# fraunhoferhhi/vvenc

Measured on AMD Instinct MI355X. Metric: frames/sec + bit-exact vs CPU, 1080p/4K 10-bit preset=faster at 1/2/4/8 GPU, higher is better.
Workload: dtype i16; 1 GPU; BASELINE configs[1]: hot-path work lists RECORDED from the reference encoder (1920x1080 10-bit synthetic clip, 65 frames, preset faster; one picture per temporal layer), replayed resident in HBM: a step = one picture's integer-ME SAD windows + sub-pel SATD stages + table calls + fused TU transform/quant lists + DMVR lists on 5 HIP streams; steps follow the GOP's 1:1:2:4:8:16 layer mix from the key; hip_streams=5, sample_pairs_per_frame=175309451, coefficients_per_frame=6951461, recorded_calls_outside_the_lists=0

## Files before the change

### vvenc_amd/csrc/dmvr.hip

```cpp
#include "common.h"

namespace {

constexpr int DP = 24;

typedef uint32_t u32x4 __attribute__( ( ext_vector_type( 4 ) ) );
typedef short dmvrS2 __attribute__( ( ext_vector_type( 2 ) ) );
__device__ __forceinline__ int dmvrDot2( uint32_t a, uint32_t b, int c ) { return __builtin_amdgcn_sdot2( __builtin_bit_cast( dmvrS2, a ), __builtin_bit_cast( dmvrS2, b ), c, false ); }
__device__ __forceinline__ uint32_t dmvrPack( int lo, int hi ) { return ( ( uint32_t ) lo & 0xffffu ) | ( ( uint32_t ) hi << 16 ); }

__device__ __forceinline__ int divMaxQ7( long long N, long long D )
{
  int sign = 0, q = 0;
  if( N < 0 ) { sign = 1; N = -N; }
  D <<= 3;
  if( N >= D ) { N -= D; q++; }
  q <<= 1;
  D >>= 1;
  if( N >= D ) { N -= D; q++; }
  q <<= 1;
  if( N >= ( D >> 1 ) ) q++;
  return sign ? -q : q;
}

VVHIP_GROUP_REDUCE( dmvrGroupMin32, ( o < v ? o : v ) )

template<int dx, int dy>
__global__ void __launch_bounds__( 256 )
dmvrRefineKernel( const int16_t* __restrict__ ref0, int stride0, const int16_t* __restrict__ ref1, int stride1, const vvhip_dmvr_item* __restrict__ items, int n,
                  int bitDepth, vvhip_dmvr_result* __restrict__ out )
{
  __shared__ __attribute__( ( aligned( 16 ) ) ) int16_t sT[4][2][22 * DP];
  __shared__ __attribute__( ( aligned( 16 ) ) ) int16_t sR[4][2][20 * DP];
  __shared__ uint32_t sCost[4][32];
  struct __attribute__( ( packed, aligned( 2 ) ) ) U16 { u32x4 v; };
  struct __attribute__( ( packed, aligned( 2 ) ) ) U4 { uint32_t v; };
  const int wv = threadIdx.x >> 6, lane = threadIdx.x & 63;
  const int q = ( int ) gridDim.x >> 3, g = ( int ) blockIdx.x < ( q << 3 ) ? ( ( int ) blockIdx.x & 7 ) * q + ( ( int ) blockIdx.x >> 3 ) : ( int ) blockIdx.x;
  const int blk = g * 4 + wv;
  if( blk >= n ) return;
  const vvhip_dmvr_item it = items[blk];
  constexpr int bw = dx + 4, bh = dy + 4, segs = ( bw + 7 ) >> 3;
  const int sh1 = 4 - ( 10 - bitDepth ), of1 = 1 << ( sh1 - 1 );
  const int16_t* s0 = ref0 + it.ref0_off - 2 * stride0 - 2;
  const int16_t* s1 = ref1 + it.ref1_off - 2 * stride1 - 2;
// ... 19 lines not shown
      u32x4 o = A[q];
      if( fxs[q] )
      {
        const uint32_t w = dmvrPack( 16 - fxs[q], fxs[q] );
        const uint32_t e[5] = { A[q].x, A[q].y, A[q].z, A[q].w, B[q] };
        uint32_t r[4];
#pragma unroll
        for( int i = 0; i < 4; i++ )
          r[i] = dmvrPack( dmvrDot2( e[i], w, of1 ) >> sh1, dmvrDot2( __builtin_amdgcn_alignbit( e[i + 1], e[i], 16 ), w, of1 ) >> sh1 );
        o.x = r[0]; o.y = r[1]; o.z = r[2]; o.w = r[3];
      }
      *reinterpret_cast<u32x4*>( &sT[wv][0][at[q]] ) = o;
    }
  }
  DMVR_SYNC();
  {
    const int perList = bh * segs, jobs = 2 * perList;
    for( int jb = lane; jb < jobs; jb += 64 )
    {
      const int list = jb >= perList, rem = jb - list * perList, y = segs == 3 ? rem / 3 : rem >> 1, x0 = ( rem - y * segs ) * 8;
      const int fx = ( list ? it.frac1_x : it.frac0_x ) & 15, fy = ( list ? it.frac1_y : it.frac0_y ) & 15;
      const u32x4 a = *reinterpret_cast<const u32x4*>( &sT[wv][list][y * DP + x0] );
      u32x4 o = a;
      if( fy )
      {
        const u32x4 b = *reinterpret_cast<const u32x4*>( &sT[wv][list][( y + 1 ) * DP + x0] );
        const int rnd = fx ? 8 : of1, sh = fx ? 4 : sh1;
        const uint32_t w = dmvrPack( 16 - fy, fy );
        const uint32_t aw[4] = { a.x, a.y, a.z, a.w }, bw_[4] = { b.x, b.y, b.z, b.w };
        uint32_t r[4];
#pragma unroll
        for( int i = 0; i < 4; i++ )
          r[i] = dmvrPack( dmvrDot2( __builtin_amdgcn_perm( bw_[i], aw[i], 0x05040100u ), w, rnd ) >> sh, dmvrDot2( __builtin_amdgcn_perm( bw_[i], aw[i], 0x07060302u ), w, rnd ) >> sh );
        o.x = r[0]; o.y = r[1]; o.z = r[2]; o.w = r[3];
      }
      else if( !fx )
      {
        const int s = 10 - bitDepth;
        const uint32_t aw[4] = { a.x, a.y, a.z, a.w };
        uint32_t r[4];
#pragma unroll
        for( int i = 0; i < 4; i++ ) r[i] = dmvrPack( ( int ) ( int16_t ) ( aw[i] & 0xffffu ) << s, ( ( int ) aw[i] >> 16 ) << s );
        o.x = r[0]; o.y = r[1]; o.z = r[2]; o.w = r[3];
      }
      o.x ^= 0x80008000u; o.y ^= 0x80008000u; o.z ^= 0x80008000u; o.w ^= 0x80008000u;
      *reinterpret_cast<u32x4*>( &sR[wv][list][y * DP + x0] ) = o;
    }
  }
  DMVR_SYNC();
  {
    constexpr int rows = dy >> 1, dw = dx >> 1, PPW = 64 / rows;
    const int r = lane & ( rows - 1 ), slot = lane / rows;
#pragma unroll
    for( int pass = 0; pass < ( 15 + PPW - 1 ) / PPW; pass++ )
    {
      const int idx = pass * PPW + slot;
      const bool valid = idx < 15;
      const int iv = valid ? idx : 7, v3 = ( iv * 11 ) >> 5, ver = v3 - 2, hor = 2 * ( iv - 3 * v3 ) - 2;
      const uint32_t* p0 = reinterpret_cast<const uint32_t*>( &sR[wv][0][( 2 + 2 * r + ver ) * DP + 2 + hor] );
      const uint32_t* p1 = reinterpret_cast<const uint32_t*>( &sR[wv][1][( 2 + 2 * r - ver ) * DP + 2 - hor] );
      uint32_t sum = 0;
// ... 67 lines not shown
  }
#undef DMVR_SYNC
}

}

extern "C" {

int vvhip_dmvr_refine_batch( vvhip_ctx* ctx, const int16_t* d_ref0, int stride0, const int16_t* d_ref1, int stride1, const vvhip_dmvr_item* d_items, int n,
                             int dx, int dy, int bit_depth, vvhip_dmvr_result* d_out )
{
  if( !ctx ) return VVHIP_E_ARG;
  if( n < 0 || ( dx != 8 && dx != 16 ) || ( dy != 8 && dy != 16 ) || bit_depth < 8 || bit_depth > 10 || ( n && ( !d_ref0 || !d_ref1 || !d_items || !d_out ) ) )
    return vvhip_fail( ctx, VVHIP_E_ARG, "vvhip_dmvr_refine_batch: sub-block %dx%d (8 or 16 per side, DMVR_SUBCU_SIZE 16) bitDepth %d (<= 10: the bilinear taps keep 10-bit precision)", dx, dy, bit_depth );
  if( n == 0 ) return VVHIP_OK;
  const dim3 grid( ( n + 3 ) / 4 ), block( 256 );
  if( dx == 16 && dy == 16 )     hipLaunchKernelGGL( ( dmvrRefineKernel<16, 16> ), grid, block, 0, ctx->stream, d_ref0, stride0, d_ref1, stride1, d_items, n, bit_depth, d_out );
  else if( dx == 16 )            hipLaunchKernelGGL( ( dmvrRefineKernel<16, 8> ), grid, block, 0, ctx->stream, d_ref0, stride0, d_ref1, stride1, d_items, n, bit_depth, d_out );
  else if( dy == 16 )            hipLaunchKernelGGL( ( dmvrRefineKernel<8, 16> ), grid, block, 0, ctx->stream, d_ref0, stride0, d_ref1, stride1, d_items, n, bit_depth, d_out );
  else                           hipLaunchKernelGGL( ( dmvrRefineKernel<8, 8> ), grid, block, 0, ctx->stream, d_ref0, stride0, d_ref1, stride1, d_items, n, bit_depth, d_out );
  VVHIP_LAUNCH_CHECK( ctx );
  return VVHIP_OK;
}

}
```

### vvenc_amd/csrc/me.hip

```cpp
#include <stdlib.h>
#ifndef VVHIP_ME_HU
#define VVHIP_ME_HU 2
#endif
#ifndef VVHIP_ME_STAGE_WAVES
#define VVHIP_ME_STAGE_WAVES 6
#endif
#ifndef VVHIP_ME_ITEM_WAVES
#define VVHIP_ME_ITEM_WAVES 8
#endif
#include <string.h>
#include <algorithm>
#include <vector>
#include "common.h"

struct vvhip_me_plan
{
  int bitDepth = 0, nCands = 0, nStages = 0, nItems = 0, nMaskItems = 0, maxPlane = 0;
  int wavesInt = 0, wavesStage = 0, wavesItem = 0, wavesItemMain = 0, ldsInt = 0, ldsStage = 0;
  int intBig = 0, ldsIntSmall = 0;
  int intLarge = 0, ldsIntMid = 0;
  bool stageAtomic = false;
  bool intSplit = false;
  bool timing = false; hipEvent_t ev[5] = { nullptr, nullptr, nullptr, nullptr, nullptr };
  int stageSetWaves[6] = { 0, 0, 0, 0, 0, 0 }, stageSetLds[6] = { 0, 0, 0, 0, 0, 0 };
  void* d_blob = nullptr;
  const void* d_intJobs = nullptr; const void* d_cands = nullptr; const void* d_candOut = nullptr; const void* d_stageJobs = nullptr; const void* d_stageOrder = nullptr; const void* d_stageWaves = nullptr;
  const void* d_items = nullptr; const void* d_itemOrder = nullptr; const void* d_itemWaves = nullptr; const void* d_tapTables = nullptr; const void* d_maskItems = nullptr;
};

namespace {

typedef uint32_t u32x2 __attribute__( ( ext_vector_type( 2 ) ) );
// ... 688 lines not shown
      for( int q = 0; q < CW / 2; q++ ) { bits |= va[q] | vb[q]; const uint32_t df = pkSub( va[q], vb[q] ); acc = ( uint32_t ) dot2( df, df, ( int ) acc ); }
    }
  }
  if( __builtin_amdgcn_ballot_w64( ( bits & 0xf000f000u ) != 0 ) == 0ull ) return acc;
  uint64_t sse = 0;
  for( int it = nIt; it > 0; it--, pa += stepA, pb += stepB )
  {
    uint32_t va[CW / 2], vb[CW / 2];
    itemChunk<CW>( pa, pb, va, vb );
#pragma unroll
    for( int q = 0; q < CW / 2; q++ ) { const int d0 = lo16( va[q] ) - lo16( vb[q] ), d1 = hi16( va[q] ) - hi16( vb[q] ); sse += ( uint64_t ) ( ( int64_t ) d0 * d0 ) + ( uint64_t ) ( ( int64_t ) d1 * d1 ); }
  }
  return sse;
}

template<bool GEN>
__device__ __forceinline__ void itemBody( const MePlanes& P, const MeArgs& a, int wave, int nItems )
{
  __shared__ const int16_t* planeL[16];
  __shared__ int strideL[16];
  const WaveSpan span = a.itemWaves[wave];
  const int lane = threadIdx.x & 63;
  if( lane < 16 ) { planeL[lane] = P.p[lane]; strideL[lane] = P.stride[lane]; }
  __builtin_amdgcn_fence( __ATOMIC_ACQ_REL, "wavefront" ); __builtin_amdgcn_wave_barrier();
  if( GEN && span.count < 0 ) { maskItemBody( a, span, nItems, planeL, strideL, lane ); return; }
  const vvhip_me_item first = a.items[span.first];
  const int w = first.width, h = first.height, func = first.func, ss = func == VVHIP_DF_SAD ? first.sub_shift : 0;
  if( func == VVHIP_DF_SAD || func == VVHIP_DF_SSE )
  {
    const int cw = w >= 8 ? 8 : ( ( !GEN || w >= 4 ) ? 4 : 2 ), lprShift = ( 31 - __builtin_clz( w ) ) - ( 31 - __builtin_clz( cw ) ), lpr = 1 << lprShift, rowsEff = h >> ss, chunks = rowsEff * lpr;
    const int lpcShift = chunks >= 64 ? 6 : 31 - __builtin_clz( chunks ), lpc = 1 << lpcShift;
    const int teams = 64 >> lpcShift, lt = lane & ( lpc - 1 ), team = lane >> lpcShift;
    for( int i0 = 0; i0 < span.count; i0 += teams )
    {
      const int ii = i0 + team;
      const bool valid = ii < span.count;
      const int idx = a.itemOrder[span.first + ( valid ? ii : 0 )];
      const vvhip_me_item it = a.items[span.first + ( valid ? ii : 0 )];
      const int16_t* po = planeL[it.org_plane] + it.org_off; const int os = strideL[it.org_plane] ? strideL[it.org_plane] : w;
      const int16_t* pc = planeL[it.cur_plane] + it.cur_off; const int cs = strideL[it.cur_plane] ? strideL[it.cur_plane] : w;
      const int r0 = lt >> lprShift, s0 = lt & ( lpr - 1 ), rowStep = lpc >> lprShift;
      const int16_t* pa = po + ( ptrdiff_t ) ( r0 << ss ) * os + s0 * cw;
      const int16_t* pb = pc + ( ptrdiff_t ) ( r0 << ss ) * cs + s0 * cw;
      const ptrdiff_t stepA = ( ptrdiff_t ) ( rowStep << ss ) * os, stepB = ( ptrdiff_t ) ( rowStep << ss ) * cs;
      const int nIt = chunks >> lpcShift;
      const bool isSad = func == VVHIP_DF_SAD;
      const uint64_t mine = cw == 8 ? itemSadSse<8>( isSad, pa, pb, stepA, stepB, nIt ) : ( ( !GEN || cw == 4 ) ? itemSadSse<4>( isSad, pa, pb, stepA, stepB, nIt ) : itemSadSse<2>( isSad, pa, pb, stepA, stepB, nIt ) );
      if( isSad ) { const uint32_t t = vvhipGroupSum32( ( uint32_t ) mine, lpc, lane ); if( valid && lt == 0 ) a.itemCost[idx] = ( uint64_t ) t << ss; }
      else        { const uint64_t t = vvhipGroupSum64( mine, lpc, lane ); if( valid && lt == 0 ) a.itemCost[idx] = t; }
    }
    return;
  }
  const int kind = GEN ? hadTileKind( w, h, func == VVHIP_DF_HAD_FAST ) : ( w == 4 ? TK_4x4 : ( ( func == VVHIP_DF_HAD_FAST && ( w & 31 ) == 0 ) ? TK_16F : TK_8x8 ) );
  if( !GEN && kind == TK_4x4 )
  {
    const int ii = lane;
    const bool valid = ii < span.count;
    const int idx = a.itemOrder[span.first + ( valid ? ii : 0 )];
    const vvhip_me_item it = a.items[span.first + ( valid ? ii : 0 )];
    const int16_t* qa = planeL[it.org_plane] + it.org_off; const int os = strideL[it.org_plane] ? strideL[it.org_plane] : w;
    const int16_t* qb = planeL[it.cur_plane] + it.cur_off; const int cs = strideL[it.cur_plane] ? strideL[it.cur_plane] : w;
    int d[16]; uint32_t sad = 0;
#pragma unroll
    for( int r = 0; r < 4; r++ )
    {
      const u32x2 x = ld8( qa + ( ptrdiff_t ) r * os ), z = ld8( qb + ( ptrdiff_t ) r * cs );
      d[4 * r] = lo16( x.x ) - lo16( z.x ); d[4 * r + 1] = hi16( x.x ) - hi16( z.x ); d[4 * r + 2] = lo16( x.y ) - lo16( z.y ); d[4 * r + 3] = hi16( x.y ) - hi16( z.y );
      if( func == VVHIP_DF_HAD_2SAD ) { sad = __builtin_amdgcn_sad_u16( x.x ^ BIAS, z.x ^ BIAS, sad ); sad = __builtin_amdgcn_sad_u16( x.y ^ BIAS, z.y ^ BIAS, sad ); }
    }
    const uint64_t tot = hadamard4x4( d ), s2 = 2ull * sad;
    if( valid ) a.itemCost[idx] = ( func == VVHIP_DF_HAD_2SAD && s2 < tot ) ? s2 : tot;
    return;
  }
  __shared__ uint32_t accAll[4][128];
  uint32_t* accL = accAll[( threadIdx.x >> 6 ) & 3];
  accL[lane] = 0; accL[64 + lane] = 0;
  __builtin_amdgcn_fence( __ATOMIC_ACQ_REL, "wavefront" ); __builtin_amdgcn_wave_barrier();
  const int PW = GEN ? tileW( kind ) : ( kind == TK_16F ? 16 : 8 ), PH = GEN ? tileH( kind ) : PW, LT = GEN ? tileLanes( kind ) : 8, log2LT = GEN ? 31 - __builtin_clz( LT ) : 3;
  const int log2TX = ( 31 - __builtin_clz( w ) ) - ( 31 - __builtin_clz( PW ) ), tilesX = 1 << log2TX, log2Slots = log2TX + ( 31 - __builtin_clz( h ) ) - ( 31 - __builtin_clz( PH ) ) + log2LT;
  const int slotsPerItem = 1 << log2Slots, total = span.count * slotsPerItem;
  for( int s0 = 0; s0 < total; s0 += 64 )
  {
    const int sl = s0 + lane;
    const bool valid = sl < total;
    const int sv = valid ? sl : 0, ii = sv >> log2Slots, rem = sv & ( slotsPerItem - 1 ), t = rem >> log2LT, r = rem & ( LT - 1 );
    const vvhip_me_item it = a.items[span.first + ii];
// ... 28 lines not shown
      }
      else
      {
        uint32_t xw[4], zw[4];
        if( GEN && kind == TK_4x8 )
        {
          const u32x2 xa = ld8( qa + ( ptrdiff_t ) ( 2 * r ) * os ), xb = ld8( qa + ( ptrdiff_t ) ( 2 * r + 1 ) * os ), za = ld8( qb + ( ptrdiff_t ) ( 2 * r ) * cs ), zb = ld8( qb + ( ptrdiff_t ) ( 2 * r + 1 ) * cs );
          xw[0] = xa.x; xw[1] = xa.y; xw[2] = xb.x; xw[3] = xb.y; zw[0] = za.x; zw[1] = za.y; zw[2] = zb.x; zw[3] = zb.y;
        }
        else
        {
          const int row = ( GEN && kind == TK_16x8 ) ? ( r & 7 ) : r, col = ( GEN && kind == TK_16x8 ) ? 8 * ( r >> 3 ) : 0;
          const u32x4 x = ld16( qa + ( ptrdiff_t ) row * os + col ), z = ld16( qb + ( ptrdiff_t ) row * cs + col );
          xw[0] = x.x; xw[1] = x.y; xw[2] = x.z; xw[3] = x.w; zw[0] = z.x; zw[1] = z.y; zw[2] = z.z; zw[3] = z.w;
        }
        if( func == VVHIP_DF_HAD_2SAD )
        {
#pragma unroll
          for( int i = 0; i < 4; i++ ) sad = __builtin_amdgcn_sad_u16( xw[i] ^ BIAS, zw[i] ^ BIAS, sad );
        }
        sres = hadTeamPk( xw, zw, r, GEN ? LT : 8, GEN ? kind : TK_8x8, lane );
      }
      if( func == VVHIP_DF_HAD_2SAD ) sad = vvhipGroupSum32( sad, GEN ? LT : 8, lane );
    }
    if( valid && r == 0 ) { atomicAdd( &accL[ii], sres ); if( func == VVHIP_DF_HAD_2SAD ) atomicAdd( &accL[64 + ii], sad ); }
  }
  __builtin_amdgcn_fence( __ATOMIC_ACQ_REL, "wavefront" ); __builtin_amdgcn_wave_barrier();
  if( lane < span.count )
  {
    const int idx = a.itemOrder[span.first + lane];
    const uint64_t tot = accL[lane], s2 = 2ull * accL[64 + lane];
    a.itemCost[idx] = ( func == VVHIP_DF_HAD_2SAD && s2 < tot ) ? s2 : tot;
  }
}

template<int K0, int K1, bool GEN>
__global__ void __launch_bounds__( 128 ) __attribute__( ( amdgpu_waves_per_eu( VVHIP_ME_STAGE_WAVES, VVHIP_ME_STAGE_WAVES ) ) )
meStageKernel( MePlanes P, MeArgs a, int firstWave, int nWaves, int ldsPerWave )
{
  extern __shared__ __attribute__( ( aligned( 16 ) ) ) int16_t meLds[];
  __shared__ uint32_t pairCost[16];
  const int wv = __builtin_amdgcn_readfirstlane( ( int ) ( threadIdx.x >> 6 ) ), wave = blockIdx.x * 2 + wv;
  if( wave < nWaves ) stageBody<K0, K1, GEN>( P, a, a.stageWaves[firstWave + wave], meLds + wv * ( ldsPerWave >> 1 ), pairCost, wv );
}

__global__ void __launch_bounds__( 256 )
meIntKernel( MePlanes P, MeArgs a, int nBig, int ldsSmall, int blockBase )
// ... 57 lines not shown
  return mePlanCreate( ctx, L, bit_depth, max_window, out );
}

int vvhip_me_plan_create_lists( vvhip_ctx* ctx, const vvhip_me_lists* lists, int bit_depth, int max_window, vvhip_me_plan** out )
{
  if( !ctx || !lists ) return VVHIP_E_ARG;
  return mePlanCreate( ctx, *lists, bit_depth, max_window, out );
}

static int mePlanCreate( vvhip_ctx* ctx, const vvhip_me_lists& L, int bit_depth, int max_window, vvhip_me_plan** out )
{
  if( !ctx || !out ) return VVHIP_E_ARG;
  *out = nullptr;
  const vvhip_me_int_job* int_jobs = L.int_jobs; const vvhip_me_cand* cands = L.cands; const vvhip_me_stage_job* stage_jobs = L.stage_jobs; const vvhip_me_item* items = L.items;
  const vvhip_me_mask_item* mask_items = L.mask_items;
  const int n_int_jobs = L.n_int_jobs, n_cands = L.n_cands, n_stage_jobs = L.n_stage_jobs, n_items = L.n_items, n_mask = L.n_mask_items;
  if( n_int_jobs < 0 || n_cands < 0 || n_stage_jobs < 0 || n_items < 0 || n_mask < 0 || ( n_int_jobs && ( !int_jobs || !cands ) ) || ( n_stage_jobs && !stage_jobs ) || ( n_items && !items ) || ( n_mask && !mask_items ) )
    return vvhip_fail( ctx, VVHIP_E_ARG, "vvhip_me_plan_create: bad lists" );
  if( n_cands >= ( 1 << 24 ) ) return vvhip_fail( ctx, VVHIP_E_ARG, "vvhip_me_plan_create: %d candidates (the schedule packs the output-list position into 24 bits)", n_cands );
  if( n_stage_jobs > ST_STAGE_MASK ) return vvhip_fail( ctx, VVHIP_E_ARG, "vvhip_me_plan_create: %d stage jobs (the schedule packs the stage index into 22 bits)", n_stage_jobs );
  if( bit_depth < 8 || bit_depth > 10 ) return vvhip_fail( ctx, VVHIP_E_UNSUPPORTED, "vvhip_me_plan_create: bit depth %d (the packed Hadamard tile covers <= 10)", bit_depth );
  if( max_window <= 0 ) max_window = 24;
  auto shapeOk = []( int w, int h, int minW, int minH ) { return isPow2( w ) && isPow2( h ) && w >= minW && h >= minH && w <= 128 && h <= 128; };

  std::vector<IntJob> ij; std::vector<PlanCand> pc; std::vector<int32_t> candOut;
  int ldsInt = 0;
  static const bool dedupe = !( getenv( "VVHIP_ME_DEDUPE" ) && atoi( getenv( "VVHIP_ME_DEDUPE" ) ) == 0 );
  static const int candCap = getenv( "VVHIP_ME_CAND_CAP" ) ? atoi( getenv( "VVHIP_ME_CAND_CAP" ) ) : 16;
  for( int i = 0; i < n_int_jobs; i++ )
  {
    const vvhip_me_int_job& s = int_jobs[i];
// ... 175 lines not shown
      }
    }
  }
  for( int k = 0, first = 0; k < 6; first += setWaves[k], k++ )
    for( int w = 0; w < setWaves[k]; w++ )
    {
      const WaveSpan& sp = stWaves[first + w];
      const int u = stOrder[sp.first];
      const vvhip_me_stage_job& s = stage_jobs[u & ST_STAGE_MASK];
      if( dealOf( s ) != 0 ) continue;
      const int sib = ( w & 1 ) ? w - 1 : w + 1;
      if( sp.count != unitsOf( s ) / 2 || sib >= setWaves[k] || stWaves[first + sib].count != sp.count || ( stOrder[stWaves[first + sib].first] & ( ST_STAGE_MASK | ( 3 << ST_VAR_SHIFT ) ) ) != ( u & ( ST_STAGE_MASK | ( 3 << ST_VAR_SHIFT ) ) ) )
        return vvhip_fail( ctx, VVHIP_E_HIP, "vvhip_me_plan_create: schedule error (the units of stage %d are not one workgroup)", u & ST_STAGE_MASK );
    }

  std::vector<int32_t> itOrder( ( size_t ) n_items + n_mask ); std::vector<WaveSpan> itWaves;
  for( int i = 0; i < n_items; i++ )
  {
    const vvhip_me_item& s = items[i];
    const bool fOk = s.func == VVHIP_DF_SAD || s.func == VVHIP_DF_SSE || s.func == VVHIP_DF_HAD || s.func == VVHIP_DF_HAD_FAST || s.func == VVHIP_DF_HAD_2SAD;
    if( !shapeOk( s.width, s.height, 2, 2 ) || !fOk || s.org_plane > 15 || s.cur_plane > 15 || s.sub_shift > 1 || ( s.sub_shift && ( s.func != VVHIP_DF_SAD || s.height < 2 ) ) )
      return vvhip_fail( ctx, VVHIP_E_ARG, "vvhip_me_plan_create: item %d (func %d, %dx%d)", i, s.func, s.width, s.height );
    itOrder[i] = i;
  }
  auto itemGen = [&]( int i ) { const auto& s = items[i]; if( s.func == VVHIP_DF_SAD || s.func == VVHIP_DF_SSE ) return s.width < 4;
                                const int kind = hadTileKind( s.width, s.height, s.func == VVHIP_DF_HAD_FAST ); return !( kind == TK_8x8 || kind == TK_16F || ( kind == TK_4x4 && s.width == 4 && s.height == 4 ) ); };
  auto itemKey = [&]( int i ) { const auto& s = items[i]; return ( itemGen( i ) ? 0l : 1l << 48 ) | ( ( long ) s.width << 32 ) | ( ( long ) s.height << 16 ) | ( s.func << 8 ) | s.sub_shift; };
  std::stable_sort( itOrder.begin(), itOrder.begin() + n_items, [&]( int a, int b ) { return itemKey( a ) > itemKey( b ); } );
  int wavesItemMain = 0;
  for( int i = 0; i < n_items; )
  {
    const vvhip_me_item& s0 = items[itOrder[i]];
    int lanesPer;
    if( s0.func == VVHIP_DF_SAD || s0.func == VVHIP_DF_SSE ) { const int cw = s0.width >= 8 ? 8 : ( s0.width >= 4 ? 4 : 2 ); lanesPer = ( s0.height >> ( s0.func == VVHIP_DF_SAD ? s0.sub_shift : 0 ) ) * ( s0.width / cw ); }
    else { const int kind = hadTileKind( s0.width, s0.height, s0.func == VVHIP_DF_HAD_FAST ); lanesPer = kind == TK_4x4 ? 1 : ( s0.width / tileW( kind ) ) * ( s0.height / tileH( kind ) ) * tileLanes( kind ); }
    if( lanesPer > 64 ) lanesPer = 64;
    const int perWave = std::max( 1, 64 / lanesPer );
    int count = 0;
    while( i + count < n_items && count < perWave && itemKey( itOrder[i + count] ) == itemKey( itOrder[i] ) ) count++;
// ... 80 lines not shown
    for( int k = 0; k < 9; k++ )
    {
      if( !( ( u.j.mask >> k ) & 1 ) ) continue;
      tx[k] = ( rxT[k] + u.j.base_qx ) * u.j.i_frac * 4; ty[k] = ( ( u.j.i_frac == 2 ? ryH[k] : ryQ[k] ) + u.j.base_qy ) * u.j.i_frac * 4;
      int v = 0; while( v < nHor && u.hx[v] != tx[k] ) v++;
      if( v == nHor ) u.hx[nHor++] = ( int16_t ) tx[k];
      var[k] = v; cnt[v]++; nPos++;
    }
    u.nHor = ( uint8_t ) nHor; u.nPos = ( uint8_t ) nPos; u.cnt0 = ( uint8_t ) cnt[0]; u.cnt1 = ( uint8_t ) cnt[1]; u.cnt2 = ( uint8_t ) cnt[2];
    int slot[3] = { 0, cnt[0], cnt[0] + cnt[1] };
    for( int k = 0; k < 9; k++ ) if( ( u.j.mask >> k ) & 1 ) u.pos[slot[var[k]]++] = k | ( ( tx[k] + 64 ) << 8 ) | ( ( ty[k] + 64 ) << 20 );
  }
  std::vector<vvhip_me_item> itSorted( n_items );
  for( int i = 0; i < n_items; i++ ) itSorted[i] = items[itOrder[i]];
  std::vector<vvhip_me_mask_item> mkSorted( n_mask );
  for( int i = 0; i < n_mask; i++ ) { mkSorted[i] = mask_items[itOrder[n_items + i]]; itOrder[n_items + i] += n_items; }
  const std::vector<int32_t> tapTab = stageTapTables( bit_depth );
  auto pad = []( size_t b ) { return ( b + 255 ) & ~( size_t ) 255; };
  const size_t bInt = pad( ij.size() * sizeof( IntJob ) ), bCand = pad( pc.size() * sizeof( PlanCand ) ), bCandO = pad( candOut.size() * 4 ), bSt = pad( stUnits.size() * sizeof( StageUnit ) ),
               bStO = pad( stOrder.size() * 4 ), bStW = pad( stWaves.size() * sizeof( WaveSpan ) ), bIt = pad( ( size_t ) n_items * sizeof( vvhip_me_item ) ), bItO = pad( itOrder.size() * 4 ),
               bItW = pad( itWaves.size() * sizeof( WaveSpan ) ), bMk = pad( mkSorted.size() * sizeof( vvhip_me_mask_item ) );
  const size_t bTap = pad( tapTab.size() * 4 );
  const size_t total = bInt + bCand + bCandO + bSt + bStO + bStW + bIt + bItO + bItW + bTap + bMk + 256;
  std::vector<char> host( total, 0 );
  size_t o = 0;
  auto put = [&]( const void* src, size_t bytes, size_t padded ) { const size_t at = o; if( bytes ) memcpy( host.data() + o, src, bytes ); o += padded; return at; };
  const size_t oInt = put( ij.data(), ij.size() * sizeof( IntJob ), bInt ), oCand = put( pc.data(), pc.size() * sizeof( PlanCand ), bCand ), oCandO = put( candOut.data(), candOut.size() * 4, bCandO ),
               oSt = put( stUnits.data(), stUnits.size() * sizeof( StageUnit ), bSt ), oStO = put( stOrder.data(), stOrder.size() * 4, bStO ),
               oStW = put( stWaves.data(), stWaves.size() * sizeof( WaveSpan ), bStW ), oIt = put( itSorted.data(), ( size_t ) n_items * sizeof( vvhip_me_item ), bIt ),
               oItO = put( itOrder.data(), itOrder.size() * 4, bItO ), oItW = put( itWaves.data(), itWaves.size() * sizeof( WaveSpan ), bItW ), oTap = put( tapTab.data(), tapTab.size() * 4, bTap ),
               oMk = put( mkSorted.data(), mkSorted.size() * sizeof( vvhip_me_mask_item ), bMk );
  vvhip_me_plan* p = new vvhip_me_plan;
  hipError_t e = hipMalloc( &p->d_blob, total );
  if( e != hipSuccess ) { delete p; return vvhip_fail( ctx, VVHIP_E_NOMEM, "vvhip_me_plan_create: hipMalloc( %zu ): %s", total, hipGetErrorString( e ) ); }
  e = hipMemcpyAsync( p->d_blob, host.data(), total, hipMemcpyHostToDevice, ctx->stream );
  if( e == hipSuccess ) e = hipStreamSynchronize( ctx->stream );
  if( e != hipSuccess ) { ( void ) hipFree( p->d_blob ); delete p; return vvhip_fail( ctx, VVHIP_E_HIP, "vvhip_me_plan_create: upload: %s", hipGetErrorString( e ) ); }
  char* b = static_cast<char*>( p->d_blob );
  p->d_intJobs = b + oInt; p->d_cands = b + oCand; p->d_candOut = b + oCandO; p->d_stageJobs = b + oSt; p->d_stageOrder = b + oStO; p->d_stageWaves = b + oStW; p->d_items = b + oIt; p->d_itemOrder = b + oItO; p->d_itemWaves = b + oItW; p->d_tapTables = b + oTap; p->d_maskItems = b + oMk;
  p->bitDepth = bit_depth; p->nCands = n_cands; p->nStages = n_stage_jobs; p->nItems = n_items; p->nMaskItems = n_mask; p->maxPlane = maxPlane; p->stageAtomic = hasAtomic;
  p->wavesInt = ( int ) ij.size(); p->wavesStage = ( int ) stWaves.size(); p->wavesItem = ( int ) itWaves.size(); p->wavesItemMain = wavesItemMain;
  p->ldsInt = ( ldsInt + 15 ) & ~15; p->ldsStage = ( ldsStage + 15 ) & ~15;
  for( int k = 0; k < 6; k++ ) { p->stageSetWaves[k] = setWaves[k]; p->stageSetLds[k] = setLds[k]; }
  p->intBig = intBig; p->ldsIntSmall = ( ldsIntSmall + 15 ) & ~15; p->intLarge = intLarge; p->ldsIntMid = ( ldsIntMid + 15 ) & ~15;
  p->intSplit = intBig > 0 && intBig < ( int ) ij.size() && p->ldsInt > 2 * 4 * p->ldsIntSmall && p->ldsInt > 32 * 1024;
  if( p->ldsInt > 160 * 1024 || p->ldsStage > 64 * 1024 )
  { ( void ) hipFree( p->d_blob ); delete p; return vvhip_fail( ctx, VVHIP_E_UNSUPPORTED, "vvhip_me_plan_create: %d / %d bytes of LDS per wave (max_window too large?)", ldsInt, ldsStage ); }
  *out = p;
  return VVHIP_OK;
}

void vvhip_me_plan_destroy( vvhip_ctx* ctx, vvhip_me_plan* plan )
{
  if( !plan ) return;
  if( ctx ) ( void ) hipStreamSynchronize( ctx->stream );
// ... 89 lines not shown
      }
      else hipLaunchKernelGGL( meIntKernel, dim3( ( unsigned ) plan->intBig ), dim3( 256 ), ( size_t ) plan->ldsInt, ctx->stream, P, a, plan->intBig, plan->ldsIntSmall, 0 );
      if( splitSmall && nSmall ) hipLaunchKernelGGL( meIntKernel, dim3( ( unsigned ) ( ( nSmall + 3 ) / 4 ) ), dim3( 256 ), ( size_t ) 4 * plan->ldsIntSmall, ctx->stream, P, a, plan->intBig, plan->ldsIntSmall, plan->intBig );
    }
  }
  if( tm ) VVHIP_CHECK_HIP( ctx, hipEventRecord( plan->ev[2], ctx->stream ) );
  if( tm ) VVHIP_CHECK_HIP( ctx, hipEventRecord( plan->ev[3], ctx->stream ) );
  if( plan->wavesItem && doItem )
  {
    const int nMain = plan->wavesItemMain, nGen = plan->wavesItem - nMain;
    static const int longSpans = getenv( "VVHIP_ME_ITEM_SPANS" ) ? atoi( getenv( "VVHIP_ME_ITEM_SPANS" ) ) : 1;
    auto launch = [&]( bool gen, int first, int n )
    {
      if( n <= 65536 )
      {
        if( gen ) hipLaunchKernelGGL( ( meItemKernel<4, true> ), dim3( ( unsigned ) ( ( n + 3 ) / 4 ) ), dim3( 256 ), 0, ctx->stream, P, a, plan->nItems, first, n, 1 );
        else      hipLaunchKernelGGL( ( meItemKernel<4, false> ), dim3( ( unsigned ) ( ( n + 3 ) / 4 ) ), dim3( 256 ), 0, ctx->stream, P, a, plan->nItems, first, n, 1 );
      }
      else
      {
        const int spw = longSpans < 1 ? 1 : longSpans, nw = ( n + spw - 1 ) / spw;
        if( gen ) hipLaunchKernelGGL( ( meItemKernel<1, true> ), dim3( ( unsigned ) nw ), dim3( 64 ), 0, ctx->stream, P, a, plan->nItems, first, n, spw );
        else      hipLaunchKernelGGL( ( meItemKernel<1, false> ), dim3( ( unsigned ) nw ), dim3( 64 ), 0, ctx->stream, P, a, plan->nItems, first, n, spw );
      }
    };
    if( nMain ) launch( false, 0, nMain );
    if( nGen ) launch( true, nMain, nGen );
  }
  VVHIP_LAUNCH_CHECK( ctx );
  if( tm ) VVHIP_CHECK_HIP( ctx, hipEventRecord( plan->ev[4], ctx->stream ) );
  return VVHIP_OK;
}

}
#endif
```

Measured before the change: 15530 frames/s.

## Early-exit DMVR on centre cost and deduplicate identical ME item calls

In DMVR, each wave first builds only the rows needed for the zero-offset SAD. If that centre cost is under the dx*dy threshold, it writes a zero refinement and returns, which skips interpolating the rest of the window and evaluating the other 14 search positions. In ME plan creation, items with the same operands are grouped so duplicate calls are computed once and the result is scattered to every output slot. A HAD item and a SAD item over the same block are also merged so one pass produces both costs. This adds host-side sorting at plan build time and indirect output lists on device, and it changes how item order is encoded, so correctness depends on the new index packing.

```diff
diff --git a/vvenc_amd/csrc/dmvr.hip b/vvenc_amd/csrc/dmvr.hip
--- a/vvenc_amd/csrc/dmvr.hip
+++ b/vvenc_amd/csrc/dmvr.hip
@@ -28,7 +28,7 @@
 template<int dx, int dy>
 __global__ void __launch_bounds__( 256 )
 dmvrRefineKernel( const int16_t* __restrict__ ref0, int stride0, const int16_t* __restrict__ ref1, int stride1, const vvhip_dmvr_item* __restrict__ items, int n,
-                  int bitDepth, vvhip_dmvr_result* __restrict__ out )
+                  int bitDepth, int centreFirst, vvhip_dmvr_result* __restrict__ out )
 {
   __shared__ __attribute__( ( aligned( 16 ) ) ) int16_t sT[4][2][22 * DP];
   __shared__ __attribute__( ( aligned( 16 ) ) ) int16_t sR[4][2][20 * DP];
@@ -78,37 +78,78 @@
     }
   }
   DMVR_SYNC();
+  const auto second = [&]( int list, int y, int x0 )
+  {
+    const int fx = ( list ? it.frac1_x : it.frac0_x ) & 15, fy = ( list ? it.frac1_y : it.frac0_y ) & 15;
+    const u32x4 a = *reinterpret_cast<const u32x4*>( &sT[wv][list][y * DP + x0] );
+    u32x4 o = a;
+    if( fy )
+    {
+      const u32x4 b = *reinterpret_cast<const u32x4*>( &sT[wv][list][( y + 1 ) * DP + x0] );
+      const int rnd = fx ? 8 : of1, sh = fx ? 4 : sh1;
+      const uint32_t w = dmvrPack( 16 - fy, fy );
+      const uint32_t aw[4] = { a.x, a.y, a.z, a.w }, bw_[4] = { b.x, b.y, b.z, b.w };
+      uint32_t r[4];
+#pragma unroll
+      for( int i = 0; i < 4; i++ )
+        r[i] = dmvrPack( dmvrDot2( __builtin_amdgcn_perm( bw_[i], aw[i], 0x05040100u ), w, rnd ) >> sh, dmvrDot2( __builtin_amdgcn_perm( bw_[i], aw[i], 0x07060302u ), w, rnd ) >> sh );
+      o.x = r[0]; o.y = r[1]; o.z = r[2]; o.w = r[3];
+    }
+    else if( !fx )
+    {
+      const int s = 10 - bitDepth;
+      const uint32_t aw[4] = { a.x, a.y, a.z, a.w };
+      uint32_t r[4];
+#pragma unroll
+      for( int i = 0; i < 4; i++ ) r[i] = dmvrPack( ( int ) ( int16_t ) ( aw[i] & 0xffffu ) << s, ( ( int ) aw[i] >> 16 ) << s );
+      o.x = r[0]; o.y = r[1]; o.z = r[2]; o.w = r[3];
+    }
+    o.x ^= 0x80008000u; o.y ^= 0x80008000u; o.z ^= 0x80008000u; o.w ^= 0x80008000u;
+    *reinterpret_cast<u32x4*>( &sR[wv][list][y * DP + x0] ) = o;
+  };
+  if( centreFirst )
+  {
+    constexpr int rows = dy >> 1, dw = dx >> 1, perList = rows * segs, restList = ( bh - rows ) * segs, ahead = 64 - 2 * perList;
+    const auto rest = [&]( int jb, int& list, int& y, int& x0 )
+    {
+      list = jb >= restList;
+      const int rem = jb - list * restList, k = segs == 3 ? rem / 3 : rem >> 1;
+      y = k < 2 ? k : k <= rows + 1 ? 2 * k - 1 : k + rows; x0 = ( rem - k * segs ) * 8;
+    };
+    {
+      int list, y, x0;
+      rest( lane - 2 * perList, list, y, x0 );
+      if( lane < 2 * perList ) { list = lane >= perList; const int rem = lane - list * perList, r = segs == 3 ? rem / 3 : rem >> 1; y = 2 + 2 * r; x0 = ( rem - r * segs ) * 8; }
+      if( lane < 2 * perList + 2 * restList ) second( list, y, x0 );
+    }
+    DMVR_SYNC();
+    uint32_t sum = 0;
+    if( lane < rows )
+    {
+      const uint32_t* p0 = reinterpret_cast<const uint32_t*>( &sR[wv][0][( 2 + 2 * lane ) * DP + 2] );
+      const uint32_t* p1 = reinterpret_cast<const uint32_t*>( &sR[wv][1][( 2 + 2 * lane ) * DP + 2] );
+#pragma unroll
+      for( int i = 0; i < dw; i++ ) sum = __builtin_amdgcn_sad_u16( p0[i], p1[i], sum );
+    }
+    const uint32_t s = ( uint32_t ) __builtin_amdgcn_readfirstlane( ( int ) vvhipGroupSum32( sum, rows, lane ) ), centre = s - ( s >> 2 );
+    if( centre < ( uint32_t ) ( dx * dy ) )
+    {
+      if( lane == 0 )
+      {
+        vvhip_dmvr_result r; r.mvd_x = 0; r.mvd_y = 0; r.pad = 0; r.min_cost = centre;
+        out[blk] = r;
+      }
+      return;
+    }
+    for( int jb = lane + ahead; jb < 2 * restList; jb += 64 ) { int list, y, x0; rest( jb, list, y, x0 ); second( list, y, x0 ); }
+  }
+  else
   {
     const int perList = bh * segs, jobs = 2 * perList;
     for( int jb = lane; jb < jobs; jb += 64 )
     {
-      const int list = jb >= perList, rem = jb - list * perList, y = segs == 3 ? rem / 3 : rem >> 1, x0 = ( rem - y * segs ) * 8;
-      const int fx = ( list ? it.frac1_x : it.frac0_x ) & 15, fy = ( list ? it.frac1_y : it.frac0_y ) & 15;
-      const u32x4 a = *reinterpret_cast<const u32x4*>( &sT[wv][list][y * DP + x0] );
-      u32x4 o = a;
-      if( fy )
-      {
-        const u32x4 b = *reinterpret_cast<const u32x4*>( &sT[wv][list][( y + 1 ) * DP + x0] );
-        const int rnd = fx ? 8 : of1, sh = fx ? 4 : sh1;
-        const uint32_t w = dmvrPack( 16 - fy, fy );
-        const uint32_t aw[4] = { a.x, a.y, a.z, a.w }, bw_[4] = { b.x, b.y, b.z, b.w };
-        uint32_t r[4];
-#pragma unroll
-        for( int i = 0; i < 4; i++ )
-          r[i] = dmvrPack( dmvrDot2( __builtin_amdgcn_perm( bw_[i], aw[i], 0x05040100u ), w, rnd ) >> sh, dmvrDot2( __builtin_amdgcn_perm( bw_[i], aw[i], 0x07060302u ), w, rnd ) >> sh );
-        o.x = r[0]; o.y = r[1]; o.z = r[2]; o.w = r[3];
-      }
-      else if( !fx )
-      {
-        const int s = 10 - bitDepth;
-        const uint32_t aw[4] = { a.x, a.y, a.z, a.w };
-        uint32_t r[4];
-#pragma unroll
-        for( int i = 0; i < 4; i++ ) r[i] = dmvrPack( ( int ) ( int16_t ) ( aw[i] & 0xffffu ) << s, ( ( int ) aw[i] >> 16 ) << s );
-        o.x = r[0]; o.y = r[1]; o.z = r[2]; o.w = r[3];
-      }
-      o.x ^= 0x80008000u; o.y ^= 0x80008000u; o.z ^= 0x80008000u; o.w ^= 0x80008000u;
-      *reinterpret_cast<u32x4*>( &sR[wv][list][y * DP + x0] ) = o;
+      const int list = jb >= perList, rem = jb - list * perList, y = segs == 3 ? rem / 3 : rem >> 1;
+      second( list, y, ( rem - y * segs ) * 8 );
     }
   }
   DMVR_SYNC();
@@ -206,11 +247,12 @@
   if( n < 0 || ( dx != 8 && dx != 16 ) || ( dy != 8 && dy != 16 ) || bit_depth < 8 || bit_depth > 10 || ( n && ( !d_ref0 || !d_ref1 || !d_items || !d_out ) ) )
     return vvhip_fail( ctx, VVHIP_E_ARG, "vvhip_dmvr_refine_batch: sub-block %dx%d (8 or 16 per side, DMVR_SUBCU_SIZE 16) bitDepth %d (<= 10: the bilinear taps keep 10-bit precision)", dx, dy, bit_depth );
   if( n == 0 ) return VVHIP_OK;
+  static const int centreFirst = []{ const char* e = getenv( "VVHIP_DMVR_CENTRE_FIRST" ); return e ? atoi( e ) != 0 : 1; }();
   const dim3 grid( ( n + 3 ) / 4 ), block( 256 );
-  if( dx == 16 && dy == 16 )     hipLaunchKernelGGL( ( dmvrRefineKernel<16, 16> ), grid, block, 0, ctx->stream, d_ref0, stride0, d_ref1, stride1, d_items, n, bit_depth, d_out );
-  else if( dx == 16 )            hipLaunchKernelGGL( ( dmvrRefineKernel<16, 8> ), grid, block, 0, ctx->stream, d_ref0, stride0, d_ref1, stride1, d_items, n, bit_depth, d_out );
-  else if( dy == 16 )            hipLaunchKernelGGL( ( dmvrRefineKernel<8, 16> ), grid, block, 0, ctx->stream, d_ref0, stride0, d_ref1, stride1, d_items, n, bit_depth, d_out );
-  else                           hipLaunchKernelGGL( ( dmvrRefineKernel<8, 8> ), grid, block, 0, ctx->stream, d_ref0, stride0, d_ref1, stride1, d_items, n, bit_depth, d_out );
+  if( dx == 16 && dy == 16 )     hipLaunchKernelGGL( ( dmvrRefineKernel<16, 16> ), grid, block, 0, ctx->stream, d_ref0, stride0, d_ref1, stride1, d_items, n, bit_depth, centreFirst, d_out );
+  else if( dx == 16 )            hipLaunchKernelGGL( ( dmvrRefineKernel<16, 8> ), grid, block, 0, ctx->stream, d_ref0, stride0, d_ref1, stride1, d_items, n, bit_depth, centreFirst, d_out );
+  else if( dy == 16 )            hipLaunchKernelGGL( ( dmvrRefineKernel<8, 16> ), grid, block, 0, ctx->stream, d_ref0, stride0, d_ref1, stride1, d_items, n, bit_depth, centreFirst, d_out );
+  else                           hipLaunchKernelGGL( ( dmvrRefineKernel<8, 8> ), grid, block, 0, ctx->stream, d_ref0, stride0, d_ref1, stride1, d_items, n, bit_depth, centreFirst, d_out );
   VVHIP_LAUNCH_CHECK( ctx );
   return VVHIP_OK;
 }
diff --git a/vvenc_amd/csrc/me.hip b/vvenc_amd/csrc/me.hip
--- a/vvenc_amd/csrc/me.hip
+++ b/vvenc_amd/csrc/me.hip
@@ -10,12 +10,13 @@
 #endif
 #include <string.h>
 #include <algorithm>
+#include <tuple>
 #include <vector>
 #include "common.h"
 
 struct vvhip_me_plan
 {
-  int bitDepth = 0, nCands = 0, nStages = 0, nItems = 0, nMaskItems = 0, maxPlane = 0;
+  int bitDepth = 0, nCands = 0, nStages = 0, nItems = 0, maskOrderAt = 0, nMaskItems = 0, maxPlane = 0;
   int wavesInt = 0, wavesStage = 0, wavesItem = 0, wavesItemMain = 0, ldsInt = 0, ldsStage = 0;
   int intBig = 0, ldsIntSmall = 0;
   int intLarge = 0, ldsIntMid = 0;
@@ -734,6 +735,23 @@
   return sse;
 }
 
+constexpr int ME_DF_HAD_SAD = 64;
+typedef int meInt2 __attribute__( ( ext_vector_type( 2 ) ) );
+__device__ __forceinline__ meInt2 itemOrderWord( const MeArgs& a, int i ) { return reinterpret_cast<const meInt2*>( a.itemOrder )[i]; }
+__device__ __forceinline__ void itemStore( const MeArgs& a, meInt2 e, uint64_t vA, uint64_t vB, int k0, int step )
+{
+  if( e.y >= -1 )
+  {
+    if( k0 == 0 ) a.itemCost[e.x] = vA;
+    if( e.y >= 0 && k0 == ( step > 1 ? 1 : 0 ) ) a.itemCost[e.y & 0x3fffffff] = ( e.y & 0x40000000 ) ? vB : vA;
+    return;
+  }
+  const int32_t* o = a.itemOrder + ( e.y & 0x7fffffff );
+  const uint32_t hdr = ( uint32_t ) o[0];
+  const int nA = ( int ) ( hdr & 0xffffu ), n = nA + ( int ) ( hdr >> 16 );
+  for( int k = k0; k < n; k += step ) a.itemCost[o[1 + k]] = k < nA ? vA : vB;
+}
+
 template<bool GEN>
 __device__ __forceinline__ void itemBody( const MePlanes& P, const MeArgs& a, int wave, int nItems )
 {
@@ -755,7 +773,7 @@
     {
       const int ii = i0 + team;
       const bool valid = ii < span.count;
-      const int idx = a.itemOrder[span.first + ( valid ? ii : 0 )];
+      const meInt2 idx = itemOrderWord( a, span.first + ( valid ? ii : 0 ) );
       const vvhip_me_item it = a.items[span.first + ( valid ? ii : 0 )];
       const int16_t* po = planeL[it.org_plane] + it.org_off; const int os = strideL[it.org_plane] ? strideL[it.org_plane] : w;
       const int16_t* pc = planeL[it.cur_plane] + it.cur_off; const int cs = strideL[it.cur_plane] ? strideL[it.cur_plane] : w;
@@ -766,17 +784,18 @@
       const int nIt = chunks >> lpcShift;
       const bool isSad = func == VVHIP_DF_SAD;
       const uint64_t mine = cw == 8 ? itemSadSse<8>( isSad, pa, pb, stepA, stepB, nIt ) : ( ( !GEN || cw == 4 ) ? itemSadSse<4>( isSad, pa, pb, stepA, stepB, nIt ) : itemSadSse<2>( isSad, pa, pb, stepA, stepB, nIt ) );
-      if( isSad ) { const uint32_t t = vvhipGroupSum32( ( uint32_t ) mine, lpc, lane ); if( valid && lt == 0 ) a.itemCost[idx] = ( uint64_t ) t << ss; }
-      else        { const uint64_t t = vvhipGroupSum64( mine, lpc, lane ); if( valid && lt == 0 ) a.itemCost[idx] = t; }
+      if( isSad ) { const uint32_t t = vvhipGroupSum32( ( uint32_t ) mine, lpc, lane ); if( valid ) itemStore( a, idx, ( uint64_t ) t << ss, 0, lt, lpc ); }
+      else        { const uint64_t t = vvhipGroupSum64( mine, lpc, lane ); if( valid ) itemStore( a, idx, t, 0, lt, lpc ); }
     }
     return;
   }
+  const bool twin = !GEN && func == ME_DF_HAD_SAD, withSad = func == VVHIP_DF_HAD_2SAD || twin;
   const int kind = GEN ? hadTileKind( w, h, func == VVHIP_DF_HAD_FAST ) : ( w == 4 ? TK_4x4 : ( ( func == VVHIP_DF_HAD_FAST && ( w & 31 ) == 0 ) ? TK_16F : TK_8x8 ) );
   if( !GEN && kind == TK_4x4 )
   {
     const int ii = lane;
     const bool valid = ii < span.count;
-    const int idx = a.itemOrder[span.first + ( valid ? ii : 0 )];
+    const meInt2 idx = itemOrderWord( a, span.first + ( valid ? ii : 0 ) );
     const vvhip_me_item it = a.items[span.first + ( valid ? ii : 0 )];
     const int16_t* qa = planeL[it.org_plane] + it.org_off; const int os = strideL[it.org_plane] ? strideL[it.org_plane] : w;
     const int16_t* qb = planeL[it.cur_plane] + it.cur_off; const int cs = strideL[it.cur_plane] ? strideL[it.cur_plane] : w;
@@ -786,10 +805,10 @@
     {
       const u32x2 x = ld8( qa + ( ptrdiff_t ) r * os ), z = ld8( qb + ( ptrdiff_t ) r * cs );
       d[4 * r] = lo16( x.x ) - lo16( z.x ); d[4 * r + 1] = hi16( x.x ) - hi16( z.x ); d[4 * r + 2] = lo16( x.y ) - lo16( z.y ); d[4 * r + 3] = hi16( x.y ) - hi16( z.y );
-      if( func == VVHIP_DF_HAD_2SAD ) { sad = __builtin_amdgcn_sad_u16( x.x ^ BIAS, z.x ^ BIAS, sad ); sad = __builtin_amdgcn_sad_u16( x.y ^ BIAS, z.y ^ BIAS, sad ); }
+      if( withSad ) { sad = __builtin_amdgcn_sad_u16( x.x ^ BIAS, z.x ^ BIAS, sad ); sad = __builtin_amdgcn_sad_u16( x.y ^ BIAS, z.y ^ BIAS, sad ); }
     }
     const uint64_t tot = hadamard4x4( d ), s2 = 2ull * sad;
-    if( valid ) a.itemCost[idx] = ( func == VVHIP_DF_HAD_2SAD && s2 < tot ) ? s2 : tot;
+    if( valid ) itemStore( a, idx, ( func == VVHIP_DF_HAD_2SAD && s2 < tot ) ? s2 : tot, sad, 0, 1 );
     return;
   }
   __shared__ uint32_t accAll[4][128];
@@ -848,23 +867,23 @@
           const u32x4 x = ld16( qa + ( ptrdiff_t ) row * os + col ), z = ld16( qb + ( ptrdiff_t ) row * cs + col );
           xw[0] = x.x; xw[1] = x.y; xw[2] = x.z; xw[3] = x.w; zw[0] = z.x; zw[1] = z.y; zw[2] = z.z; zw[3] = z.w;
         }
-        if( func == VVHIP_DF_HAD_2SAD )
+        if( withSad )
         {
 #pragma unroll
           for( int i = 0; i < 4; i++ ) sad = __builtin_amdgcn_sad_u16( xw[i] ^ BIAS, zw[i] ^ BIAS, sad );
         }
         sres = hadTeamPk( xw, zw, r, GEN ? LT : 8, GEN ? kind : TK_8x8, lane );
       }
-      if( func == VVHIP_DF_HAD_2SAD ) sad = vvhipGroupSum32( sad, GEN ? LT : 8, lane );
-    }
-    if( valid && r == 0 ) { atomicAdd( &accL[ii], sres ); if( func == VVHIP_DF_HAD_2SAD ) atomicAdd( &accL[64 + ii], sad ); }
+      if( withSad ) sad = vvhipGroupSum32( sad, GEN ? LT : 8, lane );
+    }
+    if( valid && r == 0 ) { atomicAdd( &accL[ii], sres ); if( withSad ) atomicAdd( &accL[64 + ii], sad ); }
   }
   __builtin_amdgcn_fence( __ATOMIC_ACQ_REL, "wavefront" ); __builtin_amdgcn_wave_barrier();
   if( lane < span.count )
   {
-    const int idx = a.itemOrder[span.first + lane];
+    const meInt2 idx = itemOrderWord( a, span.first + lane );
     const uint64_t tot = accL[lane], s2 = 2ull * accL[64 + lane];
-    a.itemCost[idx] = ( func == VVHIP_DF_HAD_2SAD && s2 < tot ) ? s2 : tot;
+    itemStore( a, idx, ( func == VVHIP_DF_HAD_2SAD && s2 < tot ) ? s2 : tot, accL[64 + lane], 0, 1 );
   }
 }
 
@@ -952,7 +971,8 @@
   *out = nullptr;
   const vvhip_me_int_job* int_jobs = L.int_jobs; const vvhip_me_cand* cands = L.cands; const vvhip_me_stage_job* stage_jobs = L.stage_jobs; const vvhip_me_item* items = L.items;
   const vvhip_me_mask_item* mask_items = L.mask_items;
-  const int n_int_jobs = L.n_int_jobs, n_cands = L.n_cands, n_stage_jobs = L.n_stage_jobs, n_items = L.n_items, n_mask = L.n_mask_items;
+  const int n_int_jobs = L.n_int_jobs, n_cands = L.n_cands, n_stage_jobs = L.n_stage_jobs, n_mask = L.n_mask_items;
+  int n_items = L.n_items;
   if( n_int_jobs < 0 || n_cands < 0 || n_stage_jobs < 0 || n_items < 0 || n_mask < 0 || ( n_int_jobs && ( !int_jobs || !cands ) ) || ( n_stage_jobs && !stage_jobs ) || ( n_items && !items ) || ( n_mask && !mask_items ) )
     return vvhip_fail( ctx, VVHIP_E_ARG, "vvhip_me_plan_create: bad lists" );
   if( n_cands >= ( 1 << 24 ) ) return vvhip_fail( ctx, VVHIP_E_ARG, "vvhip_me_plan_create: %d candidates (the schedule packs the output-list position into 24 bits)", n_cands );
@@ -1158,15 +1178,67 @@
         return vvhip_fail( ctx, VVHIP_E_HIP, "vvhip_me_plan_create: schedule error (the units of stage %d are not one workgroup)", u & ST_STAGE_MASK );
     }
 
-  std::vector<int32_t> itOrder( ( size_t ) n_items + n_mask ); std::vector<WaveSpan> itWaves;
   for( int i = 0; i < n_items; i++ )
   {
     const vvhip_me_item& s = items[i];
     const bool fOk = s.func == VVHIP_DF_SAD || s.func == VVHIP_DF_SSE || s.func == VVHIP_DF_HAD || s.func == VVHIP_DF_HAD_FAST || s.func == VVHIP_DF_HAD_2SAD;
     if( !shapeOk( s.width, s.height, 2, 2 ) || !fOk || s.org_plane > 15 || s.cur_plane > 15 || s.sub_shift > 1 || ( s.sub_shift && ( s.func != VVHIP_DF_SAD || s.height < 2 ) ) )
       return vvhip_fail( ctx, VVHIP_E_ARG, "vvhip_me_plan_create: item %d (func %d, %dx%d)", i, s.func, s.width, s.height );
-    itOrder[i] = i;
-  }
+  }
+  const bool merge = !( getenv( "VVHIP_ME_ITEM_MERGE" ) && atoi( getenv( "VVHIP_ME_ITEM_MERGE" ) ) == 0 );
+  std::vector<vvhip_me_item> schedItems; std::vector<int32_t> schedOut, outLists;
+  if( !merge || n_items >= ( 1 << 30 ) ) { schedItems.assign( items, items + n_items ); schedOut.resize( 2 * ( size_t ) n_items ); for( int i = 0; i < n_items; i++ ) { schedOut[2 * i] = i; schedOut[2 * i + 1] = -1; } }
+  else
+  {
+    auto opsLess = [&]( const vvhip_me_item& x, const vvhip_me_item& y )
+    { return std::make_tuple( x.width, x.height, x.org_plane, x.org_off, x.cur_plane, x.cur_off ) < std::make_tuple( y.width, y.height, y.org_plane, y.org_off, y.cur_plane, y.cur_off ); };
+    auto callLess = [&]( const vvhip_me_item& x, const vvhip_me_item& y ) { return opsLess( x, y ) || ( !opsLess( y, x ) && std::make_pair( x.func, x.sub_shift ) < std::make_pair( y.func, y.sub_shift ) ); };
+    std::vector<int32_t> byCall( n_items );
+    for( int i = 0; i < n_items; i++ ) byCall[i] = i;
+    std::stable_sort( byCall.begin(), byCall.end(), [&]( int a, int b ) { return callLess( items[a], items[b] ); } );
+    struct Group { int32_t first, nA, at, nB, atB; };
+    std::vector<Group> groups;
+    for( int i = 0; i < n_items; )
+    {
+      int j = i, had = -1, sad = -1;
+      while( j < n_items && !opsLess( items[byCall[i]], items[byCall[j]] ) )
+      {
+        int k = j;
+        while( k < n_items && k - j < 65535 && !callLess( items[byCall[j]], items[byCall[k]] ) ) k++;
+        const vvhip_me_item& s = items[byCall[j]];
+        const int kind = ( s.func == VVHIP_DF_SAD || s.func == VVHIP_DF_SSE ) ? -1 : hadTileKind( s.width, s.height, s.func == VVHIP_DF_HAD_FAST );
+        if( s.func == VVHIP_DF_HAD && had < 0 && ( kind == TK_8x8 || ( kind == TK_4x4 && s.width == 4 && s.height == 4 ) ) ) had = ( int ) groups.size();
+        if( s.func == VVHIP_DF_SAD && sad < 0 && s.sub_shift == 0 ) sad = ( int ) groups.size();
+        groups.push_back( Group{ byCall[j], k - j, j, 0, 0 } );
+        j = k;
+      }
+      if( had >= 0 && sad >= 0 )
+      {
+        Group& h = groups[had]; const Group& t = groups[sad];
+        h.first = std::min( h.first, t.first ); h.nB = t.nA; h.atB = t.at;
+        groups.erase( groups.begin() + sad );
+      }
+      i = j;
+    }
+    std::sort( groups.begin(), groups.end(), [&]( const Group& a, const Group& b ) { return a.first < b.first; } );
+    for( const Group& g : groups )
+    {
+      vvhip_me_item s = items[byCall[g.at]];
+      if( g.nB ) s.func = ME_DF_HAD_SAD;
+      schedItems.push_back( s );
+      schedOut.push_back( byCall[g.at] );
+      if( g.nA + g.nB == 1 ) { schedOut.push_back( -1 ); continue; }
+      if( g.nA + g.nB == 2 ) { schedOut.push_back( g.nB ? ( byCall[g.atB] | 0x40000000 ) : byCall[g.at + 1] ); continue; }
+      schedOut.push_back( ( int32_t ) ( 0x80000000u | ( uint32_t ) outLists.size() ) );
+      outLists.push_back( ( int32_t ) ( ( uint32_t ) g.nA | ( uint32_t ) g.nB << 16 ) );
+      for( int k = 0; k < g.nA; k++ ) outLists.push_back( byCall[g.at + k] );
+      for( int k = 0; k < g.nB; k++ ) outLists.push_back( byCall[g.atB + k] );
+    }
+  }
+  const int callerNItems = n_items;
+  items = schedItems.data(); n_items = ( int ) schedItems.size();
+  std::vector<int32_t> itOrder( ( size_t ) n_items + n_mask ); std::vector<WaveSpan> itWaves;
+  for( int i = 0; i < n_items; i++ ) itOrder[i] = i;
   auto itemGen = [&]( int i ) { const auto& s = items[i]; if( s.func == VVHIP_DF_SAD || s.func == VVHIP_DF_SSE ) return s.width < 4;
                                 const int kind = hadTileKind( s.width, s.height, s.func == VVHIP_DF_HAD_FAST ); return !( kind == TK_8x8 || kind == TK_16F || ( kind == TK_4x4 && s.width == 4 && s.height == 4 ) ); };
   auto itemKey = [&]( int i ) { const auto& s = items[i]; return ( itemGen( i ) ? 0l : 1l << 48 ) | ( ( long ) s.width << 32 ) | ( ( long ) s.height << 16 ) | ( s.func << 8 ) | s.sub_shift; };
@@ -1277,7 +1349,19 @@
   std::vector<vvhip_me_item> itSorted( n_items );
   for( int i = 0; i < n_items; i++ ) itSorted[i] = items[itOrder[i]];
   std::vector<vvhip_me_mask_item> mkSorted( n_mask );
-  for( int i = 0; i < n_mask; i++ ) { mkSorted[i] = mask_items[itOrder[n_items + i]]; itOrder[n_items + i] += n_items; }
+  for( int i = 0; i < n_mask; i++ ) { mkSorted[i] = mask_items[itOrder[n_items + i]]; itOrder[n_items + i] += callerNItems; }
+  {
+    std::vector<int32_t> dev( 2 * ( size_t ) n_items );
+    const int32_t listsAt = 2 * n_items + n_mask;
+    for( int i = 0; i < n_items; i++ )
+    {
+      const int32_t lo = schedOut[2 * itOrder[i]], hi = schedOut[2 * itOrder[i] + 1];
+      dev[2 * i] = lo; dev[2 * i + 1] = hi < -1 ? ( int32_t ) ( 0x80000000u | ( uint32_t ) ( ( hi & 0x7fffffff ) + listsAt ) ) : hi;
+    }
+    dev.insert( dev.end(), itOrder.begin() + n_items, itOrder.end() );
+    dev.insert( dev.end(), outLists.begin(), outLists.end() );
+    itOrder.swap( dev );
+  }
   const std::vector<int32_t> tapTab = stageTapTables( bit_depth );
   auto pad = []( size_t b ) { return ( b + 255 ) & ~( size_t ) 255; };
   const size_t bInt = pad( ij.size() * sizeof( IntJob ) ), bCand = pad( pc.size() * sizeof( PlanCand ) ), bCandO = pad( candOut.size() * 4 ), bSt = pad( stUnits.size() * sizeof( StageUnit ) ),
@@ -1301,7 +1385,7 @@
   if( e != hipSuccess ) { ( void ) hipFree( p->d_blob ); delete p; return vvhip_fail( ctx, VVHIP_E_HIP, "vvhip_me_plan_create: upload: %s", hipGetErrorString( e ) ); }
   char* b = static_cast<char*>( p->d_blob );
   p->d_intJobs = b + oInt; p->d_cands = b + oCand; p->d_candOut = b + oCandO; p->d_stageJobs = b + oSt; p->d_stageOrder = b + oStO; p->d_stageWaves = b + oStW; p->d_items = b + oIt; p->d_itemOrder = b + oItO; p->d_itemWaves = b + oItW; p->d_tapTables = b + oTap; p->d_maskItems = b + oMk;
-  p->bitDepth = bit_depth; p->nCands = n_cands; p->nStages = n_stage_jobs; p->nItems = n_items; p->nMaskItems = n_mask; p->maxPlane = maxPlane; p->stageAtomic = hasAtomic;
+  p->bitDepth = bit_depth; p->nCands = n_cands; p->nStages = n_stage_jobs; p->nItems = callerNItems; p->maskOrderAt = 2 * n_items; p->nMaskItems = n_mask; p->maxPlane = maxPlane; p->stageAtomic = hasAtomic;
   p->wavesInt = ( int ) ij.size(); p->wavesStage = ( int ) stWaves.size(); p->wavesItem = ( int ) itWaves.size(); p->wavesItemMain = wavesItemMain;
   p->ldsInt = ( ldsInt + 15 ) & ~15; p->ldsStage = ( ldsStage + 15 ) & ~15;
   for( int k = 0; k < 6; k++ ) { p->stageSetWaves[k] = setWaves[k]; p->stageSetLds[k] = setLds[k]; }
@@ -1421,14 +1505,14 @@
     {
       if( n <= 65536 )
       {
-        if( gen ) hipLaunchKernelGGL( ( meItemKernel<4, true> ), dim3( ( unsigned ) ( ( n + 3 ) / 4 ) ), dim3( 256 ), 0, ctx->stream, P, a, plan->nItems, first, n, 1 );
-        else      hipLaunchKernelGGL( ( meItemKernel<4, false> ), dim3( ( unsigned ) ( ( n + 3 ) / 4 ) ), dim3( 256 ), 0, ctx->stream, P, a, plan->nItems, first, n, 1 );
+        if( gen ) hipLaunchKernelGGL( ( meItemKernel<4, true> ), dim3( ( unsigned ) ( ( n + 3 ) / 4 ) ), dim3( 256 ), 0, ctx->stream, P, a, plan->maskOrderAt, first, n, 1 );
+        else      hipLaunchKernelGGL( ( meItemKernel<4, false> ), dim3( ( unsigned ) ( ( n + 3 ) / 4 ) ), dim3( 256 ), 0, ctx->stream, P, a, plan->maskOrderAt, first, n, 1 );
       }
       else
       {
         const int spw = longSpans < 1 ? 1 : longSpans, nw = ( n + spw - 1 ) / spw;
-        if( gen ) hipLaunchKernelGGL( ( meItemKernel<1, true> ), dim3( ( unsigned ) nw ), dim3( 64 ), 0, ctx->stream, P, a, plan->nItems, first, n, spw );
-        else      hipLaunchKernelGGL( ( meItemKernel<1, false> ), dim3( ( unsigned ) nw ), dim3( 64 ), 0, ctx->stream, P, a, plan->nItems, first, n, spw );
+        if( gen ) hipLaunchKernelGGL( ( meItemKernel<1, true> ), dim3( ( unsigned ) nw ), dim3( 64 ), 0, ctx->stream, P, a, plan->maskOrderAt, first, n, spw );
+        else      hipLaunchKernelGGL( ( meItemKernel<1, false> ), dim3( ( unsigned ) nw ), dim3( 64 ), 0, ctx->stream, P, a, plan->maskOrderAt, first, n, spw );
       }
     };
     if( nMain ) launch( false, 0, nMain );
```

Result: no change. 15500 frames/s (-0.2%).
